# ZINZINBIN/Optimal-Control-1D-Electrostatic-Plasma

Hardware: AMD Instinct MI355X
Metric: particle-steps/sec (N×envs×steps) at N=1e6, Ng=256; % HBM roofline (higher is better)
Workload: dtype f64

## Files before the change

optimal-control-1d-electrostatic-plasma_amd/csrc/host_plan.h:

```cpp
#pragma once

#include <cmath>
#include <cstddef>
#include <cstdint>
#include <string>

#include "picstep.h"

#include "pic_limits.h"

enum Format : int { FMT_F64 = 0, FMT_F32 = 1, FMT_U32 = 2 };

struct LaunchPlan {
  int fmt = FMT_F64;
  int acc_kind = PIC_ACC_FIX64;
  int vec = 2;
  size_t esz = 8;
  long long ld = 0;
  long long chunk = 0;
  int nblk = 0;
  int R = 1;
  int fg = 42;
  int S = 1;
  double magic = 0;
  size_t sweep_lds = 0, solve_lds = 0;
  bool resident = false;
  int res_ppt = 0, res_nw = 0, res_R = 1;
  bool res_lean = false;
  size_t res_lds = 0;
  size_t res_carry_bytes = 0;
  double dx = 0, scale = 0;
  double cs[4]{}, ds[4]{};
  bool light_inner_steps = false;
  bool readonly_auto = false;
  size_t sweep_lds_rc = 0;
  bool v_separate = false;
  bool h_part_at_create = false;
  bool h_fields = false;
};

static inline void yoshida_coefficients(double (&c)[4], double (&d)[4]) {
  const double cbrt2 = std::pow(2.0, 1.0 / 3.0);
  const double w0 = (-1) * cbrt2 / (2 - cbrt2);
  const double w1 = 1 / (2 - cbrt2);
  c[0] = c[3] = 0.5 * w1;
  c[1] = c[2] = 0.5 * (w0 + w1);
  d[0] = 0.0;
  d[1] = d[3] = w1;
  d[2] = w0;
}

static inline int plan_fail(std::string* err, const std::string& msg) {
  if (err) *err = msg;
  return PIC_EINVAL;
}

static inline int check_config(const pic_config& c, std::string* err) {
  const pic_config* cfg = &c;
  if (cfg->N < 1 || cfg->Ng < 4 || cfg->num_envs < 1 || !(cfg->L > 0) || !(cfg->dt > 0) || !(cfg->n0 > 0))
    return plan_fail(err, "pic_create: need N>=1, Ng>=4, num_envs>=1, L>0, dt>0, n0>0");
  if (cfg->N > (1ll << 36)) return plan_fail(err, "pic_create: N > 2^36");
  if (cfg->num_envs > 65535) return plan_fail(err, "pic_create: num_envs > 65535");
  if (cfg->env_index_base < 0) return plan_fail(err, "pic_create: env_index_base < 0");
  if (cfg->particle_dtype != PIC_F64 && cfg->particle_dtype != PIC_F32)
    return plan_fail(err, "pic_create: particle_dtype must be PIC_F64 or PIC_F32");
  if (cfg->position_dtype != PIC_POS_FLOAT && cfg->position_dtype != PIC_POS_FIXED32)
    return plan_fail(err, "pic_create: position_dtype must be PIC_POS_FLOAT or PIC_POS_FIXED32");
  if (cfg->position_dtype == PIC_POS_FIXED32 && cfg->particle_dtype != PIC_F32)
    return plan_fail(err, "pic_create: 32-bit fixed-point positions go with float32 particles");
  if (cfg->accum_dtype < PIC_ACC_AUTO || cfg->accum_dtype > PIC_ACC_F64)
    return plan_fail(err, "pic_create: accum_dtype must be PIC_ACC_AUTO, _FIX64, _PACKED or _F64");
  if (cfg->interpol != PIC_CIC && cfg->interpol != PIC_TSC)
    return plan_fail(err, "pic_create: interpol must be PIC_CIC or PIC_TSC");
  if (cfg->accum_dtype == PIC_ACC_PACKED && cfg->particle_dtype != PIC_F32)
    return plan_fail(err, "pic_create: the packed accumulator needs float32 particles");
  if (cfg->accum_dtype == PIC_ACC_PACKED && cfg->interpol != PIC_CIC)
    return plan_fail(err, "pic_create: the packed accumulator is CIC only");
  if (cfg->placement != PIC_PLACE_AUTO && cfg->placement != PIC_PLACE_OFF)
    return plan_fail(err, "pic_create: placement must be PIC_PLACE_AUTO or PIC_PLACE_OFF");
  if (cfg->placement_ms < 0) return plan_fail(err, "pic_create: placement_ms < 0");
  if (cfg->accum_dtype == PIC_ACC_F64 && cfg->particle_dtype != PIC_F64)
    return plan_fail(err, "pic_create: the float64 accumulator needs float64 particles");
  return PIC_OK;
}

static inline int plan_launch(const pic_config& c, int ncu, LaunchPlan* p, std::string* err) {
  const pic_config* cfg = &c;
  *p = LaunchPlan{};
  p->fmt = cfg->particle_dtype == PIC_F64 ? FMT_F64 : (cfg->position_dtype == PIC_POS_FIXED32 ? FMT_U32 : FMT_F32);
  p->acc_kind = cfg->accum_dtype;
  if (p->acc_kind == PIC_ACC_AUTO)
    p->acc_kind = (cfg->particle_dtype == PIC_F32 && cfg->interpol == PIC_CIC) ? PIC_ACC_PACKED : PIC_ACC_FIX64;
  p->esz = cfg->particle_dtype == PIC_F64 ? 8 : 4;
  p->vec = cfg->particle_dtype == PIC_F64 ? 2 : 4;
  p->dx = cfg->L / cfg->Ng;
  p->scale = cfg->n0 * cfg->L / (double)cfg->N / p->dx;
  yoshida_coefficients(p->cs, p->ds);
  p->ld = (cfg->N + 63) / 64 * 64;
  int lg = 0;
  while ((1ll << lg) < cfg->N + 1) ++lg;
  p->fg = 62 - lg > 50 ? 50 : 62 - lg;
  p->magic = std::ldexp(1.5, 52 - p->fg);

  const long long tile = (long long)BLOCK * p->vec;
  long long nblk = cfg->blocks_per_env;
  if (nblk <= 0) {
    const long long target_total = 8192;
    nblk = (target_total + cfg->num_envs - 1) / cfg->num_envs;
    const bool small = (double)cfg->N * cfg->num_envs <= 4.0e6 && cfg->N <= 131072;
    long long tiles_min = small ? 1 : 8;
    if (!small && (cfg->N + 8 * tile - 1) / (8 * tile) * cfg->num_envs < 256) tiles_min = 4;
    long long max_by_work = (cfg->N + tiles_min * tile - 1) / (tiles_min * tile);
    if (small && max_by_work > 64) max_by_work = 64;
    if (nblk > max_by_work) nblk = max_by_work;
    if (nblk < 1) nblk = 1;
    const long long by10 = (cfg->N + 10 * tile - 1) / (10 * tile);
    if (!small && nblk < by10) nblk = by10;
    if (!small) {
      const long long by4 = (cfg->N + 4 * tile - 1) / (4 * tile);
      if (nblk * cfg->num_envs < 6ll * ncu) {
        for (long long k = 2; k <= 6; ++k) {
          long long c = k * ncu / cfg->num_envs;
          if (c > by4) c = by4;
          if (c >= nblk || c == by4) { nblk = c; break; }
        }
      }
    }
  }
  {
    const long long cap = (1ll << 27) - tile;
    if (nblk < (cfg->N + cap - 1) / cap) nblk = (cfg->N + cap - 1) / cap;
  }
  if (p->acc_kind == PIC_ACC_PACKED) {
    const long long cap = (1ll << 20) - tile;
    if (nblk < (cfg->N + cap - 1) / cap) nblk = (cfg->N + cap - 1) / cap;
  }
  long long chunk = (cfg->N + nblk - 1) / nblk;
  chunk = (chunk + tile - 1) / tile * tile;
  nblk = (cfg->N + chunk - 1) / chunk;
  if (nblk > 65535) return plan_fail(err, "pic_create: blocks_per_env too large");
  p->chunk = chunk;
  p->nblk = (int)nblk;
  p->light_inner_steps = 2.0 * (double)cfg->num_envs * (double)p->ld * (double)p->esz >= 256.0 * 1048576.0;
  p->readonly_auto = p->light_inner_steps;
  p->S = 1;
  while (p->S < 4 && nblk / (2 * p->S) >= 8 && (long long)cfg->num_envs * 2 * p->S <= 32) p->S *= 2;

  const size_t stride = (size_t)cfg->Ng + 2;
  p->R = 1;
  p->sweep_lds = 2 * p->R * stride * 8 + stride * p->esz;
  p->solve_lds = 2 * (size_t)cfg->Ng * sizeof(double);
  if (p->sweep_lds + stride * p->esz + kSweepStaticLds <= kLdsLimit) p->sweep_lds_rc = p->sweep_lds + stride * p->esz;
  else p->readonly_auto = false;
  if (p->sweep_lds + kSweepStaticLds > kLdsLimit) {
    const long long max_ng = (long long)((kLdsLimit - kSweepStaticLds) / (2 * p->R * 8 + p->esz)) - 2;
    return plan_fail(err, "pic_create: Ng too large for the LDS-resident mesh (at most " + std::to_string(max_ng) +
                                     " cells with this particle dtype)");
  }
  {
    static const int shapes[4][3] = {{8, 4, 2048}, {8, 8, 4096}, {8, 10, 5120}, {8, 16, 8192}};
    for (const auto& sh : shapes)
      if (cfg->N <= sh[2]) { p->res_nw = sh[0]; p->res_ppt = sh[1]; break; }
    p->res_R = 1;
    auto need = [&](int R) { return (size_t)2 * R * stride * 8 + 4 * (size_t)cfg->Ng * 8 + stride * p->esz; };
    while (p->res_R > 1 && need(p->res_R) > 48 * 1024) p->res_R >>= 1;
    p->res_lds = need(p->res_R);
    const bool possible = p->res_nw != 0 && p->res_lds + kResidentStaticLds <= kLdsLimit && p->acc_kind != PIC_ACC_F64;
    if (cfg->blocks_per_env < 0 && !possible) {
      const long long max_ng = (long long)((kLdsLimit - kResidentStaticLds - 2 * (2 * 8 + p->esz)) / (2 * 8 + p->esz + 4 * 8));
      return plan_fail(err, "pic_create: the resident schedule needs N <= 8192, Ng <= " + std::to_string(max_ng) +
                                       " (this particle dtype) and an integer accumulator");
    }
    const bool worth = cfg->N <= 5120 || cfg->num_envs >= 32;
    p->resident = possible && (cfg->blocks_per_env < 0 || (cfg->blocks_per_env == 0 && worth));
    p->res_lean = (cfg->num_envs > ncu && p->res_ppt <= 10) || (cfg->interpol == PIC_TSC && p->res_ppt == 16);
  }
  if (p->resident && !p->res_lean && p->res_ppt <= 10 && p->esz == 8 && cfg->num_envs <= 32)
    p->res_carry_bytes = (size_t)cfg->num_envs * p->res_nw * 64 * p->res_ppt * (sizeof(int) + (cfg->interpol == PIC_TSC ? 4 : 2) * p->esz);
  p->v_separate = 2 * ((size_t)cfg->num_envs * p->ld * p->esz) >= ((size_t)256 << 20) && cfg->placement != PIC_PLACE_OFF;
  p->h_part_at_create = 2 * (size_t)cfg->num_envs * cfg->N * p->esz <= ((size_t)4 << 20);
  p->h_fields = (size_t)cfg->num_envs * cfg->Ng * sizeof(double) <= ((size_t)256 << 10);
  return PIC_OK;
}
```

optimal-control-1d-electrostatic-plasma_amd/csrc/pic_device.h:

```cpp
#pragma once
#include <hip/hip_runtime.h>

#include <cmath>
#include <cstdint>
#include <type_traits>

#include "picstep.h"
#include "pic_limits.h"

namespace {

#ifndef PIC_STAMP
#define PIC_STAMP(slot) ((void)0)
#define PIC_STAMP_LOADS(slot) ((void)0)
#endif

constexpr int kInlineDoubles = 32;
struct InlineDoubles { double v[kInlineDoubles]; };

template <typename T>
__device__ __forceinline__ T kernarg_at(size_t offset) {
#if defined(__HIP_DEVICE_COMPILE__)
  using KP = const __attribute__((address_space(4))) char*;
  KP ka = (KP)__builtin_amdgcn_kernarg_segment_ptr();
  asm volatile("" : "+s"(ka));
  T out;
  __builtin_memcpy(&out, (const __attribute__((address_space(4))) T*)(ka + offset), sizeof(T));
  return out;
#else
  (void)offset;
  return T{};
#endif
}

template <typename T>
__device__ __forceinline__ const T* kernarg_ptr(size_t offset) {
#if defined(__HIP_DEVICE_COMPILE__)
  using KP = const __attribute__((address_space(4))) char*;
  KP ka = (KP)__builtin_amdgcn_kernarg_segment_ptr();
  return (const T*)(const char*)(ka + offset);
#else
  (void)offset;
  return nullptr;
#endif
}

template <int BYTES>
__device__ __forceinline__ void kernarg_warm() {
#if defined(__HIP_DEVICE_COMPILE__)
  using KP = const __attribute__((address_space(4))) unsigned*;
  KP ka = (KP)__builtin_amdgcn_kernarg_segment_ptr();
  unsigned w = 0;
#pragma unroll
  for (int line = 1; line < (BYTES + 63) / 64; ++line) w |= ka[line * 16];
  asm volatile("" ::"s"(w));
#endif
}

enum Stage : int {
  ST_A = 0,
  ST_B = 1,
  ST_C = 2,
  ST_D = 3,
  ST_REFRESH = 4,
  ST_PROBE = 5,
  ST_B2 = 6,
  ST_D2 = 7,
  ST_SE = 8,
  ST_FE = 9,
  ST_VK = 10,
  ST_VM = 11,
  ST_C_RO = 12,
  ST_D_RC = 13,
  ST_D2_RC = 14
};

using acc_t = long long;

__device__ __forceinline__ acc_t acc_row_sum(const acc_t* __restrict__ row, int j, int S, long long sub) {
  const acc_t* p = row + j;
  acc_t t = 0;
  int s = 0;
  for (; s + 4 <= S; s += 4) {
    const acc_t r0 = p[0]; p += sub;
    const acc_t r1 = p[0]; p += sub;
    const acc_t r2 = p[0]; p += sub;
    const acc_t r3 = p[0]; p += sub;
    t += (r0 + r1) + (r2 + r3);
  }
  for (; s < S; ++s) { t += p[0]; p += sub; }
  return t;
}

struct SweepArgs {
  long long N;
  long long ld;
  long long chunk;
  int Ng;
  int nblk;
  int R;
  int reverse;
  int fg;
  int S;
  int act_inline;
  long long sub;
  double magic;
  double L, dx, rdx, dt;
  double c_prev, c_cur, d_cur, c_next, d_prev;
  double scale, n0;
  double to_units;
  double N_over_L;
};

struct SolveArgs {
  long long N;
  long long sub;
  int Ng;
  int nblk;
  int fg;
  int S;
  double L, dx, n0;
  double scale;
  double N_over_L;
};

struct AccRequest { acc_t r[4]; };
__device__ __forceinline__ AccRequest acc_row_request(const acc_t* __restrict__ row, int j, int S, long long sub) {
  AccRequest q;
#pragma unroll
  for (int s = 0; s < 4; ++s) q.r[s] = row[(size_t)(s < S ? s : 0) * sub + j];
  return q;
}
__device__ __forceinline__ acc_t acc_row_finish(const AccRequest& q, int S) {
  return (q.r[0] + (S > 1 ? q.r[1] : 0)) + ((S > 2 ? q.r[2] : 0) + (S > 3 ? q.r[3] : 0));
}

struct Control {
  const double* ext;
  const double* act;
  const double* basis;
  int M;
};

__device__ __forceinline__ double actuator_field(const double* __restrict__ bc, const double* __restrict__ bs,
                                                 const double* __restrict__ a, int j, int M) {
  double c = 0.0, s = 0.0;
  for (int m = 0; m < M; ++m) c += bc[(size_t)j * M + m] * a[m];
  for (int m = 0; m < M; ++m) s += bs[(size_t)j * M + m] * a[M + m];
  return c + s;
}

typedef double pic_v2d __attribute__((ext_vector_type(2)));
typedef float pic_v4f __attribute__((ext_vector_type(4)));
typedef unsigned pic_v4u __attribute__((ext_vector_type(4)));

struct PosF64 { using X = double;   using V = double; using W = double; using XV = pic_v2d; using VV = pic_v2d; static constexpr int VEC = 2; static constexpr bool kFixed = false; };
struct PosF32 { using X = float;    using V = float;  using W = float;  using XV = pic_v4f; using VV = pic_v4f; static constexpr int VEC = 4; static constexpr bool kFixed = false; };
struct PosU32 { using X = unsigned; using V = float;  using W = float;  using XV = pic_v4u; using VV = pic_v4f; static constexpr int VEC = 4; static constexpr bool kFixed = true; };

template <typename VT>
__device__ __forceinline__ VT stream_load(const VT* p) { return *p; }

struct StreamOut {
  __amdgpu_buffer_rsrc_t rsrc;
  __device__ explicit StreamOut(void* base) : rsrc(__builtin_amdgcn_make_buffer_rsrc(base, 0, 0x7fffffff, 0x00020000)) {}
  template <typename VT>
  __device__ __forceinline__ void store(int off, VT v) const {
    static_assert(sizeof(VT) == 16, "particle tiles are 16 bytes per lane");
    typedef unsigned pic_v4raw __attribute__((ext_vector_type(4)));
    pic_v4raw w;
    __builtin_memcpy(&w, &v, 16);
    __builtin_amdgcn_raw_buffer_store_b128(w, rsrc, off, 0, 16);
  }
};

template <typename P>
struct Consts {
  typename P::W L, dx, rdx, dt, c_prev, c_cur, d_cur, c_next, d_prev;
  float to_units;
  double magic;
  int Ng;
  __device__ explicit Consts(const SweepArgs& a)
      : L((typename P::W)a.L), dx((typename P::W)a.dx), rdx((typename P::W)a.rdx), dt((typename P::W)a.dt),
        c_prev((typename P::W)a.c_prev), c_cur((typename P::W)a.c_cur), d_cur((typename P::W)a.d_cur),
        c_next((typename P::W)a.c_next), d_prev((typename P::W)a.d_prev), to_units((float)a.to_units), magic(a.magic), Ng(a.Ng) {}
  __device__ Consts(double L_, double dx_, int Ng_)
      : L((typename P::W)L_), dx((typename P::W)dx_), rdx((typename P::W)1 / (typename P::W)dx_), dt(0), c_prev(0),
        c_cur(0), d_cur(0), c_next(0), d_prev(0), to_units((float)(4294967296.0 / L_)), magic(0), Ng(Ng_) {}
};

template <typename T>
__device__ __noinline__ T wrap_periodic_far(T q, T L) {
  T r = fmod(q, L);
  if (r < T(0)) {
    r += L;
    if (r >= L) r = T(0);
  } else if (r == T(0)) {
    r = T(0);
  }
  return r;
}

template <typename T>
__device__ __forceinline__ T wrap_periodic(T q, T L, unsigned& bad) {
  if (__builtin_amdgcn_ballot_w64(!(q > T(0) && q < L)) == 0) return q;
  T up = q + L;
  up = (up >= L) ? T(0) : up;
  T r = (q <= T(0)) ? up : q;
  r = (q >= L) ? q - L : r;
  if (__builtin_expect(!(r >= T(0) && r < L), 0)) {
    r = wrap_periodic_far(q, L);
    if (!(r >= T(0) && r < L)) {
      bad += 1u;
      r = T(0);
    }
  }
  return r;
}

template <typename T>
__device__ __forceinline__ T div_dx(T a, T dx, T rdx) {
  T q0 = a * rdx;
  T rem = fma(-q0, dx, a);
  return fma(rem, rdx, q0);
}

template <typename P, int SHAPE>
__device__ __forceinline__ void locate_in_box(typename P::X xw, const Consts<P>& k, int& j, typename P::W (&w)[3], unsigned& frac) {
  using T = typename P::W;
  static_assert(!P::kFixed, "fixed-point positions need no wrap: locate() is the whole of it");
  frac = 0u;
  T jf = floor(div_dx(xw, k.dx, k.rdx));
  j = (int)jf;
  if ((unsigned)j >= (unsigned)k.Ng) j = 0;
  if (SHAPE == PIC_CIC) {
    w[0] = div_dx((jf + T(1)) * k.dx - xw, k.dx, k.rdx);
    w[1] = div_dx(xw - jf * k.dx, k.dx, k.rdx);
    w[2] = T(0);
  } else {
    T d = div_dx(xw - jf * k.dx, k.dx, k.rdx);
    T a = T(1.5) - d, b = d - T(1), c = d - T(0.5);
    w[0] = T(0.5) * (a * a);
    w[1] = T(0.75) - b * b;
    w[2] = T(0.5) * (c * c);
  }
}

template <typename P, int SHAPE>
__device__ __forceinline__ void locate(typename P::X q, const Consts<P>& k, typename P::X& xw, int& j,
                                       typename P::W (&w)[3], unsigned& frac, unsigned& bad) {
  using T = typename P::W;
  if constexpr (P::kFixed) {
    xw = q;
    j = (int)__umulhi(q, (unsigned)k.Ng);
    frac = q * (unsigned)k.Ng;
    const T d = (T)frac * T(2.3283064365386963e-10);
    if (SHAPE == PIC_CIC) {
      w[1] = d;
      w[0] = T(1) - d;
      w[2] = T(0);
    } else {
      T a = T(1.5) - d, b = d - T(1), c = d - T(0.5);
      w[0] = T(0.5) * (a * a);
      w[1] = T(0.75) - b * b;
      w[2] = T(0.5) * (c * c);
    }
  } else {
    xw = wrap_periodic(q, k.L, bad);
    locate_in_box<P, SHAPE>(xw, k, j, w, frac);
  }
}

template <typename P>
__device__ __forceinline__ double pos_to_length(typename P::X q, double L) {
  if constexpr (P::kFixed) return (double)q * (L * 2.3283064365386963e-10);
  else return (double)q;
}

template <typename P>
__device__ __forceinline__ typename P::X pos_from_length(double xs, double L, unsigned& bad) {
  if constexpr (P::kFixed) {
    double r = xs - floor(xs / L) * L;
    if (!(r >= 0.0 && r < L)) { if (!(r == L)) bad += 1u; r = 0.0; }
    return (unsigned)((unsigned long long)rint(r / L * 4294967296.0) & 0xFFFFFFFFull);
  } else {
    return (typename P::X)xs;
  }
}

template <typename P>
__device__ __forceinline__ typename P::X drift(typename P::X q, typename P::V p, typename P::W c, const Consts<P>& k,
                                               unsigned& bad) {
  using T = typename P::W;
  if constexpr (P::kFixed) {
    const float d = ((c * (T)p) * k.dt) * k.to_units;
    if (!(fabsf(d) < 2147483648.0f)) bad += 1u;
    return q + (unsigned)__float2int_rn(d);
  } else {
    return q + (c * (T)p) * k.dt;
  }
}

template <typename T, int SHAPE>
__device__ __forceinline__ T gather_field(const T* __restrict__ Es, int j, const T (&w)[3]) {
  T e = w[0] * Es[j] + w[1] * Es[j + 1];
  if (SHAPE == PIC_TSC) e = e + w[2] * Es[j + 2];
  return e;
}

struct fix_t { unsigned long long v; };
constexpr int FX_FRAC = 24;
constexpr int FX_LOW = 44;

__device__ __forceinline__ acc_t to_fixed(double w, double magic) {
  return __double_as_longlong(w + magic) - __double_as_longlong(magic);
}

template <typename A, typename P, int SHAPE>
__device__ __forceinline__ void deposit(A* __restrict__ acc, int j, const typename P::W (&w)[3], unsigned frac,
                                        double magic) {
  if constexpr (std::is_same<A, fix_t>::value) {
    static_assert(SHAPE == PIC_CIC, "the packed accumulator is CIC only");
    unsigned long long lo;
    if constexpr (P::kFixed) {
      lo = (frac >> 8) + ((frac >> 7) & 1u);
    } else {
      const float wr = fminf(fmaxf((float)w[1], 0.0f), 1.0f);
      lo = (unsigned long long)(unsigned)(wr * (float)(1u << FX_FRAC) + 0.5f);
    }
    atomicAdd(reinterpret_cast<unsigned long long*>(acc) + j, (1ull << FX_LOW) + lo);
  } else if constexpr (std::is_same<A, acc_t>::value) {
    unsigned long long* a = reinterpret_cast<unsigned long long*>(acc);
    atomicAdd(a + j, (unsigned long long)to_fixed((double)w[0], magic));
    atomicAdd(a + j + 1, (unsigned long long)to_fixed((double)w[1], magic));
    if (SHAPE == PIC_TSC) atomicAdd(a + j + 2, (unsigned long long)to_fixed((double)w[2], magic));
  } else {
    atomicAdd(&acc[j], (A)w[0]);
    atomicAdd(&acc[j + 1], (A)w[1]);
    if (SHAPE == PIC_TSC) atomicAdd(&acc[j + 2], (A)w[2]);
  }
}

template <int CTRL, int ROW_MASK = 0xF>
__device__ __forceinline__ double dpp_add(double v) {
  const int lo = __builtin_amdgcn_update_dpp(0, __double2loint(v), CTRL, ROW_MASK, 0xF, true);
  const int hi = __builtin_amdgcn_update_dpp(0, __double2hiint(v), CTRL, ROW_MASK, 0xF, true);
  return v + __hiloint2double(hi, lo);
}

__device__ __forceinline__ double wave_incl_scan(double v) {
  v = dpp_add<0x111>(v);
  v = dpp_add<0x112>(v);
  v = dpp_add<0x114>(v);
  v = dpp_add<0x118>(v);
  v = dpp_add<0x142, 0xA>(v);
  v = dpp_add<0x143, 0xC>(v);
  return v;
}

__device__ __forceinline__ double wave_sum(double v) {
  v = wave_incl_scan(v);
  const int lo = __builtin_amdgcn_readlane(__double2loint(v), 63);
  const int hi = __builtin_amdgcn_readlane(__double2hiint(v), 63);
  return __hiloint2double(hi, lo);
}

template <int NW>
__device__ __forceinline__ double block_excl_scan(double v, double* ws, double& total) {
  const int lane = threadIdx.x & 63, w = threadIdx.x >> 6;
  double inc = wave_incl_scan(v);
  if (lane == 63) ws[w] = inc;
  __syncthreads();
  double off = 0.0, tot = 0.0;
  for (int i = 0; i < NW; ++i) {
    double s = ws[i];
    if (i < w) off += s;
    tot += s;
  }
  __syncthreads();
  total = tot;
  return off + (inc - v);
}

template <int NW>
__device__ __forceinline__ double block_sum(double v, double* ws) {
  double w = wave_sum(v);
  if ((threadIdx.x & 63) == 0) ws[threadIdx.x >> 6] = w;
  __syncthreads();
  double s = 0.0;
  for (int i = 0; i < NW; ++i) s += ws[i];
  __syncthreads();
  return s;
}

template <int NW>
__device__ __forceinline__ void block_sum2(double a, double b, double* ws, double& sa, double& sb) {
  const double wa = wave_sum(a), wb = wave_sum(b);
  if ((threadIdx.x & 63) == 0) {
    ws[threadIdx.x >> 6] = wa;
    ws[NW + (threadIdx.x >> 6)] = wb;
  }
  __syncthreads();
  sa = 0.0;
  sb = 0.0;
  for (int i = 0; i < NW; ++i) {
    sa += ws[i];
    sb += ws[NW + i];
  }
  __syncthreads();
}

template <int NW>
__device__ __forceinline__ void mesh_mode(const double* __restrict__ E, const double* __restrict__ twc,
                                          const double* __restrict__ tws, int Ng, double* __restrict__ ws, double& re,
                                          double& im) {
  double sr = 0.0, si = 0.0;
  int t0 = threadIdx.x;
  asm volatile("" : "+v"(t0));
  for (int j = t0; j < Ng; j += NW * 64) {
    const double e = E[j];
    sr += e * twc[j];
    si -= e * tws[j];
  }
  double a, b;
  block_sum2<NW>(sr, si, ws, a, b);
  re = a / Ng * 2.0;
  im = b / Ng * 2.0;
}

struct Feedback {
  const double* tw;
  int rows;
  int M;
  double* act_out;
  double* act_hist;
  const double* gain;
  double* modes;
  double* modes_hist;
};

__device__ __forceinline__ double gain_row(const double* __restrict__ g, const double* __restrict__ m, int n) {
  double acc = 0.0;
  bool any = false;
  for (int k = 0; k < n; ++k) {
    const double gk = g[k];
    if (gk != 0.0) {
      const double t = gk * m[k];
      acc = any ? acc + t : t;
      any = true;
    }
  }
  return acc;
}

template <int NW>
__device__ __forceinline__ void feedback_action(const double* __restrict__ E, const Feedback& fb, int env, int Ng,
                                                double* __restrict__ ws, double* __restrict__ a_lds) {
  const size_t r = (size_t)env * 2 * fb.M;
  for (int m = 0; m < fb.M; ++m) {
    double re, im;
    mesh_mode<NW>(E, fb.tw + (size_t)m * Ng, fb.tw + ((size_t)fb.rows + m) * Ng, Ng, ws, re, im);
    if (threadIdx.x == 0) {
      if (fb.gain) {
        double* mv = a_lds ? a_lds : fb.modes + r;
        mv[m] = re; mv[fb.M + m] = im;
        if (fb.modes_hist) { fb.modes_hist[r + m] = re; fb.modes_hist[r + fb.M + m] = im; }
        continue;
      }
      const double c = -re, s = im;
      if (a_lds) { a_lds[m] = c; a_lds[fb.M + m] = s; }
      if (fb.act_out) { fb.act_out[r + m] = c; fb.act_out[r + fb.M + m] = s; }
      if (fb.act_hist) { fb.act_hist[r + m] = c; fb.act_hist[r + fb.M + m] = s; }
    }
  }
  if (fb.gain) {
    __syncthreads();
    const int n = 2 * fb.M;
    int i = threadIdx.x;
    asm volatile("" : "+v"(i));
    const double a = i < n ? gain_row(fb.gain + (r + i) * n, a_lds ? a_lds : fb.modes + r, n) : 0.0;
    if (a_lds) __syncthreads();
    if (i < n) {
      if (a_lds) a_lds[i] = a;
      if (fb.act_out) fb.act_out[r + i] = a;
      if (fb.act_hist) fb.act_hist[r + i] = a;
    }
  }
}

__device__ __forceinline__ void scan_fields(double* __restrict__ sb, double* __restrict__ sp, int Ng, double dx,
                                            double* __restrict__ slot, int wave = 0) {
  if ((int)(threadIdx.x >> 6) != wave) return;
  const int lane = threadIdx.x & 63;
  const int m = (Ng + 63) / 64;
  const int lo = min(lane * m, Ng), hi = min(lo + m, Ng);
  double loc = 0.0;
  for (int j = lo; j < hi; ++j) loc += sb[j];
  double run = wave_incl_scan(loc) - loc;
  loc = 0.0;
  for (int j = lo; j < hi; ++j) {
    run += sb[j];
    const double g = run * dx;
    sb[j] = g;
    loc += g;
  }
  const double gmean = wave_sum(loc) / (double)Ng;
  if (lane == 0) slot[0] = gmean;
  if (sp) {
    loc = 0.0;
    for (int j = lo; j < hi; ++j) loc += (sb[j] - gmean) * dx;
    run = wave_incl_scan(loc) - loc;
    double ploc = 0.0;
    for (int j = lo; j < hi; ++j) {
      sp[j] = run;
      ploc += run;
      run += (sb[j] - gmean) * dx;
    }
    ploc = wave_sum(ploc);
    if (lane == 0) slot[1] = ploc / (double)Ng;
  }
}

struct SolveOut {
  const double* ext;
  double *E, *phi;
  double *KE, *PE, *PEr;
  double* hist;
  int num_envs;
  Feedback fb;
};

template <int NW>
__device__ __forceinline__ void solve_block(const SolveOut& o, int env, int Ng, double dx, double N_over_L, double ke_share,
                                            double* __restrict__ sb, double* __restrict__ se, double* __restrict__ ws,
                                            double* __restrict__ slot) {
  constexpr int NT = NW * 64;
  const int tid = threadIdx.x;
  const size_t row = (size_t)env * Ng;
  scan_fields(sb, o.phi ? se : nullptr, Ng, dx, slot);
  __syncthreads();
  const double gmean = slot[0];
  const double pmean = o.phi ? slot[1] : 0.0;
  double e2 = 0.0;
  for (int j = tid; j < Ng; j += NT) {
    const double gp = sb[j] - gmean;
    const double gm = sb[j == 0 ? Ng - 1 : j - 1] - gmean;
    const double E = -0.5 * (gp + gm);
    const double Et = o.ext ? E + o.ext[row + j] : E;
    if (o.E) o.E[row + j] = Et;
    e2 += Et * Et;
    if (o.phi) o.phi[row + j] = se[j] - pmean;
  }
  double S, K;
  block_sum2<NW>(e2, ke_share, ws, S, K);
  if (tid == 0) {
    const double pe = 0.5 * S * dx;
    if (o.PEr) o.PEr[env] = pe;
    if (o.PE) o.PE[env] = pe * N_over_L;
    if (o.KE) o.KE[env] = 0.5 * K;
    if (o.hist) {
      o.hist[env] = 0.5 * K;
      o.hist[o.num_envs + env] = pe * N_over_L;
      o.hist[2 * (size_t)o.num_envs + env] = pe;
    }
  }
  if (o.fb.M > 0) feedback_action<NW>(o.E + row, o.fb, env, Ng, ws, nullptr);
}

}
```

optimal-control-1d-electrostatic-plasma_amd/csrc/pic_sweep.h:

```cpp
#pragma once
#include "pic_device.h"
#include "pic_solve.h"

namespace {

template <typename T, int OFF>
__device__ __forceinline__ void prologue_field(const acc_t* __restrict__ acc_in, const AccRequest& first, int S, long long sub,
                                               const Control& ctl, double* __restrict__ ext_out, int Ng, double unit, double scale,
                                               double n0, double dx, double* __restrict__ sb, double* __restrict__ xt,
                                               double* __restrict__ slot, T* __restrict__ Es) {
  const int tid = threadIdx.x;
  if (ctl.act)
    for (int j = tid; j < Ng; j += BLOCK) {
      const double e = actuator_field(ctl.basis, ctl.basis + (size_t)Ng * ctl.M, ctl.act, j, ctl.M);
      xt[j] = e;
      if (ext_out) ext_out[j] = e;
    }
  if (tid < Ng) sb[tid] = ((double)acc_row_finish(first, S) * unit) * scale - n0;
  for (int j = tid + BLOCK; j < Ng; j += BLOCK)
    sb[j] = ((double)acc_row_sum(acc_in, j, S, sub) * unit) * scale - n0;
  __syncthreads();
  PIC_STAMP(3);
  scan_fields(sb, nullptr, Ng, dx, slot);
  __syncthreads();
  PIC_STAMP(4);
  const double gmean = slot[0];
  for (int i = tid; i < Ng + 2; i += BLOCK) {
    int node = i - OFF;
    node = node < 0 ? node + Ng : (node >= Ng ? node - Ng : node);
    const double gp = sb[node] - gmean;
    const double gm = sb[node == 0 ? Ng - 1 : node - 1] - gmean;
    double E = -0.5 * (gp + gm);
    if (ctl.act) E += xt[node];
    else if (ctl.ext) E += ctl.ext[node];
    Es[i] = (T)E;
  }
  __syncthreads();
  PIC_STAMP(5);
}

template <typename P, int SHAPE>
__device__ __forceinline__ void substage(typename P::X& q, typename P::V& p, const typename P::W* __restrict__ Es,
                                         typename P::W d, typename P::W c, const Consts<P>& k, unsigned& bad) {
  using T = typename P::W;
  T w[3];
  typename P::X xw;
  int j;
  unsigned frac;
  locate<P, SHAPE>(q, k, xw, j, w, frac, bad);
  const T E = gather_field<T, SHAPE>(Es, j, w);
  p = p + (typename P::V)((d * (-E)) * k.dt);
  q = drift<P>(q, p, c, k, bad);
}

template <typename P, typename A, int SHAPE, int STAGE>
__device__ __forceinline__ void push_one(typename P::X& xq, typename P::V& vp, const typename P::W* __restrict__ Es,
                                         const typename P::W* __restrict__ Es2, A* __restrict__ acc, A* __restrict__ acc2,
                                         const Consts<P>& k, double& ke, unsigned& bad) {
  constexpr bool kC = (STAGE == ST_C || STAGE == ST_C_RO);
  constexpr bool kRC = (STAGE == ST_D_RC || STAGE == ST_D2_RC);
  constexpr bool kD = (STAGE == ST_D || STAGE == ST_D_RC);
  constexpr bool kD2 = (STAGE == ST_D2 || STAGE == ST_D2_RC);
  using T = typename P::W;
  T w[3];
  typename P::X xw;
  int j;
  unsigned frac;
  typename P::X q = xq;
  typename P::V p = vp;
  if (kRC) {
    unsigned again = 0u;
    substage<P, SHAPE>(q, p, Es2, k.d_prev, k.c_prev, k, again);
  }
  if (STAGE == ST_B2) {
    if constexpr (P::kFixed) locate<P, SHAPE>(q, k, xw, j, w, frac, bad);
    else locate_in_box<P, SHAPE>(q, k, j, w, frac);
    deposit<A, P, SHAPE>(acc2, j, w, frac, k.magic);
  }
  if (STAGE == ST_A) {
    q = drift<P>(q, p, k.c_cur, k, bad);
  } else if (STAGE == ST_B || STAGE == ST_B2 || kC || kD || kD2) {
    if (STAGE == ST_B || STAGE == ST_B2) q = drift<P>(q, p, k.c_prev, k, bad);
    substage<P, SHAPE>(q, p, Es, k.d_cur, k.c_cur, k, bad);
  }
  if (kD2) {
    if constexpr (P::kFixed) xw = q;
    else xw = wrap_periodic(q, k.L, bad);
  } else {
    locate<P, SHAPE>(q, k, xw, j, w, frac, bad);
    deposit<A, P, SHAPE>(acc, j, w, frac, k.magic);
  }
  if (kD || kD2 || STAGE == ST_REFRESH) {
    q = xw;
    ke += (double)p * (double)p;
    const typename P::X qn = drift<P>(q, p, k.c_next, k, bad);
    typename P::X xn;
    locate<P, SHAPE>(qn, k, xn, j, w, frac, bad);
    deposit<A, P, SHAPE>(acc2, j, w, frac, k.magic);
  }
  xq = q;
  vp = p;
}

template <typename P, typename A, int SHAPE, int STAGE>
__device__ __forceinline__ void push_scheme(typename P::X& xq, typename P::V& vp, const typename P::W* __restrict__ Es,
                                            A* __restrict__ acc, const Consts<P>& k, double& ke, unsigned& bad) {
  using T = typename P::W;
  using V = typename P::V;
  T w[3];
  typename P::X xw;
  int j;
  unsigned frac;
  typename P::X q = xq;
  V p = vp;
  locate<P, SHAPE>(q, k, xw, j, w, frac, bad);
  const T E = gather_field<T, SHAPE>(Es, j, w);
  if (STAGE == ST_FE) {
    q = drift<P>(xw, p, k.c_cur, k, bad);
    p = p + (V)((k.d_cur * (-E)) * k.dt);
  } else {
    p = p + (V)((k.d_cur * (-E)) * k.dt);
    if (STAGE == ST_VK || STAGE == ST_VM) {
      q = xw;
      ke += (double)p * (double)p;
    }
    if (STAGE == ST_VM) p = p + (V)((k.d_cur * (-E)) * k.dt);
    if (STAGE != ST_VK) q = drift<P>(q, p, k.c_cur, k, bad);
  }
  if (STAGE != ST_VK) {
    locate<P, SHAPE>(q, k, xw, j, w, frac, bad);
    deposit<A, P, SHAPE>(acc, j, w, frac, k.magic);
    if (STAGE != ST_VM) {
      q = xw;
      ke += (double)p * (double)p;
    }
  }
  xq = q;
  vp = p;
}

template <typename A, int SHAPE>
__device__ __forceinline__ acc_t mesh_node_sum(const A* __restrict__ acc_all, int R, int stride, int Ng, int fg, int c) {
  constexpr int OFF = (SHAPE == PIC_TSC) ? 1 : 0;
  if constexpr (std::is_same<A, fix_t>::value) {
    const unsigned long long* a = reinterpret_cast<const unsigned long long*>(acc_all);
    const int cm = c == 0 ? Ng - 1 : c - 1;
    unsigned long long own = 0ull, left = 0ull;
    for (int r = 0; r < R; ++r) {
      own += a[(size_t)r * stride + c];
      left += a[(size_t)r * stride + cm];
    }
    const long long mask = (1ll << FX_LOW) - 1;
    const long long q = ((long long)(own >> FX_LOW) << FX_FRAC) - ((long long)own & mask) + ((long long)left & mask);
    return q << (fg - FX_FRAC);
  } else {
    A s = A(0);
    for (int r = 0; r < R; ++r) {
      const A* ar = acc_all + (size_t)r * stride;
      A t = ar[c + OFF];
      if (SHAPE == PIC_CIC) {
        if (c == 0) t += ar[Ng];
      } else {
        if (c == 0) t += ar[Ng + 1];
        if (c == Ng - 1) t += ar[0];
      }
      s += t;
    }
    if constexpr (std::is_same<A, acc_t>::value) return s;
    else return __double2ll_rn(ldexp((double)s, fg));
  }
}

template <typename A, int SHAPE>
__device__ __forceinline__ void flush_mesh(const A* __restrict__ acc_all, int R, int stride, int Ng, int fg,
                                           acc_t* __restrict__ row) {
  unsigned long long* out = reinterpret_cast<unsigned long long*>(row);
  for (int c = threadIdx.x; c < Ng; c += BLOCK) {
    const acc_t q = mesh_node_sum<A, SHAPE>(acc_all, R, stride, Ng, fg, c);
    if (q) atomicAdd(out + c, (unsigned long long)q);
  }
}

struct SweepIO {
  const acc_t* acc_in;
  Control ctl;
  double* ext_out;
  const double* next_act;
  acc_t* acc_out;
  acc_t* acc_out2;
  acc_t* zero0;
  acc_t* zero1;
  double* ke_part;
  unsigned long long* bad;
  SolveIO post;
  double* e2;
};

constexpr size_t kSweepInlineOffset = 2 * sizeof(void*) + sizeof(SweepIO) + sizeof(SweepArgs);
static_assert(sizeof(SweepIO) % 8 == 0 && sizeof(SweepArgs) % 8 == 0, "arguments lie back to back");

template <typename P, typename A, int SHAPE, int STAGE>
__global__ __launch_bounds__(BLOCK) void sweep_kernel(typename P::X* __restrict__ x, typename P::V* __restrict__ v,
                                                      SweepIO io, SweepArgs a, InlineDoubles act_inline) {
  constexpr int OFF = (SHAPE == PIC_TSC) ? 1 : 0;
  constexpr int VEC = P::VEC;
  using T = typename P::W;
  using XV = typename P::XV;
  using VV = typename P::VV;
  constexpr bool kIsB = (STAGE == ST_B || STAGE == ST_B2), kIsC = (STAGE == ST_C || STAGE == ST_C_RO);
  constexpr bool kRC = (STAGE == ST_D_RC || STAGE == ST_D2_RC);
  constexpr bool kIsD = (STAGE == ST_D || STAGE == ST_D2 || kRC);
  constexpr bool kScheme = (STAGE >= ST_SE && STAGE <= ST_VM);
  constexpr bool kGather = (kIsB || kIsC || kIsD || kScheme);
  constexpr bool kStore = ((kGather && STAGE != ST_C_RO) || STAGE == ST_REFRESH);
  constexpr bool kStoreV = kGather && STAGE != ST_C_RO;
  constexpr bool kAhead = !kStore;
  constexpr bool kReadV = (STAGE != ST_PROBE);
  constexpr bool kFirst = (STAGE != ST_D2 && STAGE != ST_D2_RC && STAGE != ST_VK);
  constexpr bool kDual = (kIsD || STAGE == ST_REFRESH || STAGE == ST_B2);
  constexpr bool kEnergy = (kIsD || STAGE == ST_REFRESH || kScheme);

  extern __shared__ __align__(16) unsigned char smem_raw[];
  const int Ng = a.Ng;
  const int stride = Ng + 2;
  A* acc_all = reinterpret_cast<A*>(smem_raw);
  A* acc2_all = acc_all + (size_t)a.R * stride;
  T* Es = reinterpret_cast<T*>(smem_raw + (size_t)2 * a.R * stride * sizeof(A));
  T* Es2 = Es + stride;
  __shared__ double red[2 * WAVES];
  __shared__ double slot[2];
  static_assert(sizeof(red) + sizeof(slot) == kSweepStaticLds, "pic_create adds the static LDS to the dynamic part it sizes");
  PIC_STAMP(0);

  if (kIsC && blockIdx.x == (unsigned)a.nblk) {
    SolveIO post = kernarg_at<SolveIO>(2 * sizeof(void*) + offsetof(SweepIO, post));
    post.out.fb = Feedback{};
    solve_environment(post, blockIdx.y, Ng, a.nblk, a.fg, a.S, a.sub, a.scale, a.n0, a.dx, a.N_over_L, smem_raw, red, slot);
    return;
  }

  const int tid = threadIdx.x;
  const int env = a.reverse ? (int)gridDim.y - 1 - (int)blockIdx.y : (int)blockIdx.y;
  const int blk = a.reverse ? a.nblk - 1 - (int)blockIdx.x : (int)blockIdx.x;

  typename P::X* xe = x + (size_t)env * a.ld;
  typename P::V* ve = v + (size_t)env * a.ld;
  const long long step = (long long)BLOCK * VEC;
  const long long begin = (long long)blk * a.chunk;
  long long end = begin + a.chunk;
  if (end > a.N) end = a.N;
  long long i = begin + (long long)tid * VEC;
  AccRequest first_node{};
  if (kGather) first_node = acc_row_request(io.acc_in + (size_t)env * Ng, tid < Ng ? tid : Ng - 1, a.S, a.sub);
  const long long i_first = (i + VEC <= end) ? i : 0;
  XV xv = stream_load(reinterpret_cast<const XV*>(xe + i_first));
  VV vv = {};
  if (kReadV) vv = stream_load(reinterpret_cast<const VV*>(ve + i_first));
  PIC_STAMP(2);

  bool clear_first = true;
  if (kGather) {
    Control ctl = io.ctl;
    if (ctl.ext) ctl.ext += (size_t)env * Ng;
    if (a.act_inline) ctl.act = kernarg_ptr<double>(kSweepInlineOffset);
    if (ctl.act) ctl.act += (size_t)env * 2 * ctl.M;
    else {
      for (int c = tid; c < a.R * stride; c += BLOCK) acc_all[c] = A{};
      clear_first = false;
    }
    prologue_field<T, OFF>(io.acc_in + (size_t)env * Ng, first_node, a.S, a.sub, ctl,
                           (io.ext_out && blk == 0) ? io.ext_out + (size_t)env * Ng : nullptr, Ng, ldexp(1.0, -a.fg), a.scale, a.n0, a.dx,
                           reinterpret_cast<double*>(acc2_all), reinterpret_cast<double*>(smem_raw), slot, Es);
  }
  if (STAGE == ST_C_RO && blk == 0)
    for (int c = tid; c < stride; c += BLOCK) io.e2[(size_t)env * stride + c] = (double)Es[c];
  if (kRC)
    for (int c = tid; c < stride; c += BLOCK) Es2[c] = (T)io.e2[(size_t)env * stride + c];
  if (kIsD && io.next_act && io.ext_out && blk == 0) {
    const Control ctl = io.ctl;
    for (int j = tid; j < Ng; j += BLOCK)
      io.ext_out[(size_t)env * Ng + j] = actuator_field(ctl.basis, ctl.basis + (size_t)Ng * ctl.M, io.next_act + (size_t)env * 2 * ctl.M, j, ctl.M);
  }
  if (clear_first) for (int c = tid; c < a.R * stride; c += BLOCK) acc_all[c] = A{};
  if (kDual) for (int c = tid; c < a.R * stride; c += BLOCK) acc2_all[c] = A{};
  if (blk < a.S) {
    const size_t z = (size_t)blk * a.sub + (size_t)env * Ng;
    if (io.zero0) for (int c = tid; c < Ng; c += BLOCK) io.zero0[z + c] = 0;
    if (io.zero1) for (int c = tid; c < Ng; c += BLOCK) io.zero1[z + c] = 0;
  }
  if (clear_first || kDual) __syncthreads();
  PIC_STAMP(6);

  const int rep = (tid >> 6) & (a.R - 1);
  A* acc = acc_all + (size_t)rep * stride;
  A* acc2 = acc2_all + (size_t)rep * stride;
  const Consts<P> k(a);

  double ke = 0.0;
  unsigned bad = 0u;
  [[maybe_unused]] int tile = 0;
  const StreamOut xout(xe + begin), vout(ve + begin);
  while (i + VEC <= end) {
    PIC_STAMP_LOADS(8 + 2 * tile);
    [[maybe_unused]] XV xv_next;
    [[maybe_unused]] VV vv_next = {};
    if constexpr (kAhead) {
      const long long i_next = (i + step + VEC <= end) ? i + step : 0;
      xv_next = stream_load(reinterpret_cast<const XV*>(xe + i_next));
      if (kReadV) vv_next = stream_load(reinterpret_cast<const VV*>(ve + i_next));
    }
    typename P::X* xs = reinterpret_cast<typename P::X*>(&xv);
    typename P::V* vs = reinterpret_cast<typename P::V*>(&vv);
#pragma unroll
    for (int c = 0; c < VEC; ++c) {
      typename P::V pv = kReadV ? vs[c] : typename P::V(0);
      if constexpr (kScheme) push_scheme<P, A, SHAPE, STAGE>(xs[c], pv, Es, acc, k, ke, bad);
      else push_one<P, A, SHAPE, STAGE>(xs[c], pv, Es, Es2, acc, acc2, k, ke, bad);
      if (kReadV) vs[c] = pv;
    }
    if (kStore) {
      xout.store((int)((i - begin) * (long long)sizeof(typename P::X)), xv);
      if (kStoreV) vout.store((int)((i - begin) * (long long)sizeof(typename P::V)), vv);
    }
    PIC_STAMP(9 + 2 * tile);
    ++tile;
    i += step;
    if constexpr (kAhead) {
      xv = xv_next;
      vv = vv_next;
    } else if (i + VEC <= end) {
      xv = stream_load(reinterpret_cast<const XV*>(xe + i));
      if (kReadV) vv = stream_load(reinterpret_cast<const VV*>(ve + i));
    }
  }
  for (long long c = i; c < end; ++c) {
    typename P::X xq = xe[c];
    typename P::V pv = kReadV ? ve[c] : typename P::V(0);
    if constexpr (kScheme) push_scheme<P, A, SHAPE, STAGE>(xq, pv, Es, acc, k, ke, bad);
    else push_one<P, A, SHAPE, STAGE>(xq, pv, Es, Es2, acc, acc2, k, ke, bad);
    if (kStore) {
      xe[c] = xq;
      if (kStoreV) ve[c] = pv;
    }
  }
  __syncthreads();
  PIC_STAMP(24);

  const size_t sub_row = (size_t)(blk % a.S) * a.sub + (size_t)env * Ng;
  if (kFirst) flush_mesh<A, SHAPE>(acc_all, a.R, stride, Ng, a.fg, io.acc_out + sub_row);
  if (kDual) flush_mesh<A, SHAPE>(acc2_all, a.R, stride, Ng, a.fg, io.acc_out2 + sub_row);
  PIC_STAMP(25);

  if (kEnergy) {
    double w = wave_sum(ke);
    if ((tid & 63) == 0) red[tid >> 6] = w;
    __syncthreads();
    if (tid == 0) {
      double s = 0.0;
      for (int c = 0; c < WAVES; ++c) s += red[c];
      io.ke_part[(size_t)env * a.nblk + blk] = s;
    }
  }
  if (bad) atomicAdd(io.bad, (unsigned long long)bad);
  PIC_STAMP_LOADS(26);
}

}
```

Measured before the change: 76.71 billion.

## Trim particle push inner loop: unfolded CIC index, cheaper fixed-point convert, double-buffered tile loads

Adds a ping-pong double-buffered main loop that loads the next particle tile through scalar base plus vector lane offset addressing while pushing the current one, replacing the per-tile prefetch loop for most tiles. For CIC with non-fixed accumulators it skips folding the out-of-range cell index, and instead has the mesh flush pick up the extra ghost node. It also makes to_fixed subtract only the high 32-bit word of the magic constant, with a host check that the low word is zero. The periodic wrap is restructured to a single return path. A profiling summary script is included as well.

Measured after the change: 77.64 billion (median of 6 runs). +1.2%, better.

```diff
diff --git a/optimal-control-1d-electrostatic-plasma_amd/csrc/host_plan.h b/optimal-control-1d-electrostatic-plasma_amd/csrc/host_plan.h
--- a/optimal-control-1d-electrostatic-plasma_amd/csrc/host_plan.h
+++ b/optimal-control-1d-electrostatic-plasma_amd/csrc/host_plan.h
@@ -3,6 +3,7 @@
 #include <cmath>
 #include <cstddef>
 #include <cstdint>
+#include <cstring>
 #include <string>
 
 #include "picstep.h"
@@ -101,6 +102,11 @@
   while ((1ll << lg) < cfg->N + 1) ++lg;
   p->fg = 62 - lg > 50 ? 50 : 62 - lg;
   p->magic = std::ldexp(1.5, 52 - p->fg);
+  {
+    std::uint64_t bits;
+    std::memcpy(&bits, &p->magic, sizeof(bits));
+    if ((bits & 0xffffffffull) != 0) return plan_fail(err, "pic_create: the fixed-point magic has a non-zero low word");
+  }
 
   const long long tile = (long long)BLOCK * p->vec;
   long long nblk = cfg->blocks_per_env;
diff --git a/optimal-control-1d-electrostatic-plasma_amd/csrc/pic_device.h b/optimal-control-1d-electrostatic-plasma_amd/csrc/pic_device.h
--- a/optimal-control-1d-electrostatic-plasma_amd/csrc/pic_device.h
+++ b/optimal-control-1d-electrostatic-plasma_amd/csrc/pic_device.h
@@ -203,16 +203,18 @@
 
 template <typename T>
 __device__ __forceinline__ T wrap_periodic(T q, T L, unsigned& bad) {
-  if (__builtin_amdgcn_ballot_w64(!(q > T(0) && q < L)) == 0) return q;
-  T up = q + L;
-  up = (up >= L) ? T(0) : up;
-  T r = (q <= T(0)) ? up : q;
-  r = (q >= L) ? q - L : r;
-  if (__builtin_expect(!(r >= T(0) && r < L), 0)) {
-    r = wrap_periodic_far(q, L);
-    if (!(r >= T(0) && r < L)) {
-      bad += 1u;
-      r = T(0);
+  T r = q;
+  if (__builtin_amdgcn_ballot_w64(!(q > T(0) && q < L)) != 0) {
+    T up = q + L;
+    up = (up >= L) ? T(0) : up;
+    r = (q <= T(0)) ? up : q;
+    r = (q >= L) ? q - L : r;
+    if (__builtin_expect(!(r >= T(0) && r < L), 0)) {
+      r = wrap_periodic_far(q, L);
+      if (!(r >= T(0) && r < L)) {
+        bad += 1u;
+        r = T(0);
+      }
     }
   }
   return r;
@@ -225,14 +227,14 @@
   return fma(rem, rdx, q0);
 }
 
-template <typename P, int SHAPE>
+template <typename P, int SHAPE, bool FOLD = true>
 __device__ __forceinline__ void locate_in_box(typename P::X xw, const Consts<P>& k, int& j, typename P::W (&w)[3], unsigned& frac) {
   using T = typename P::W;
   static_assert(!P::kFixed, "fixed-point positions need no wrap: locate() is the whole of it");
   frac = 0u;
   T jf = floor(div_dx(xw, k.dx, k.rdx));
   j = (int)jf;
-  if ((unsigned)j >= (unsigned)k.Ng) j = 0;
+  if (FOLD && (unsigned)j >= (unsigned)k.Ng) j = 0;
   if (SHAPE == PIC_CIC) {
     w[0] = div_dx((jf + T(1)) * k.dx - xw, k.dx, k.rdx);
     w[1] = div_dx(xw - jf * k.dx, k.dx, k.rdx);
@@ -246,7 +248,7 @@
   }
 }
 
-template <typename P, int SHAPE>
+template <typename P, int SHAPE, bool FOLD = true>
 __device__ __forceinline__ void locate(typename P::X q, const Consts<P>& k, typename P::X& xw, int& j,
                                        typename P::W (&w)[3], unsigned& frac, unsigned& bad) {
   using T = typename P::W;
@@ -267,7 +269,7 @@
     }
   } else {
     xw = wrap_periodic(q, k.L, bad);
-    locate_in_box<P, SHAPE>(xw, k, j, w, frac);
+    locate_in_box<P, SHAPE, FOLD>(xw, k, j, w, frac);
   }
 }
 
@@ -312,8 +314,12 @@
 constexpr int FX_FRAC = 24;
 constexpr int FX_LOW = 44;
 
+typedef int pic_v2i __attribute__((ext_vector_type(2)));
+
 __device__ __forceinline__ acc_t to_fixed(double w, double magic) {
-  return __double_as_longlong(w + magic) - __double_as_longlong(magic);
+  pic_v2i s = __builtin_bit_cast(pic_v2i, w + magic);
+  s.y -= __builtin_bit_cast(pic_v2i, magic).y;
+  return __builtin_bit_cast(acc_t, s);
 }
 
 template <typename A, typename P, int SHAPE>
diff --git a/optimal-control-1d-electrostatic-plasma_amd/csrc/pic_sweep.h b/optimal-control-1d-electrostatic-plasma_amd/csrc/pic_sweep.h
--- a/optimal-control-1d-electrostatic-plasma_amd/csrc/pic_sweep.h
+++ b/optimal-control-1d-electrostatic-plasma_amd/csrc/pic_sweep.h
@@ -39,7 +39,10 @@
   PIC_STAMP(5);
 }
 
-template <typename P, int SHAPE>
+template <typename A, int SHAPE>
+constexpr bool kFoldIndex = !(SHAPE == PIC_CIC && !std::is_same<A, fix_t>::value);
+
+template <typename P, int SHAPE, bool FOLD>
 __device__ __forceinline__ void substage(typename P::X& q, typename P::V& p, const typename P::W* __restrict__ Es,
                                          typename P::W d, typename P::W c, const Consts<P>& k, unsigned& bad) {
   using T = typename P::W;
@@ -47,7 +50,7 @@
   typename P::X xw;
   int j;
   unsigned frac;
-  locate<P, SHAPE>(q, k, xw, j, w, frac, bad);
+  locate<P, SHAPE, FOLD>(q, k, xw, j, w, frac, bad);
   const T E = gather_field<T, SHAPE>(Es, j, w);
   p = p + (typename P::V)((d * (-E)) * k.dt);
   q = drift<P>(q, p, c, k, bad);
@@ -61,6 +64,7 @@
   constexpr bool kRC = (STAGE == ST_D_RC || STAGE == ST_D2_RC);
   constexpr bool kD = (STAGE == ST_D || STAGE == ST_D_RC);
   constexpr bool kD2 = (STAGE == ST_D2 || STAGE == ST_D2_RC);
+  constexpr bool kFold = kFoldIndex<A, SHAPE>;
   using T = typename P::W;
   T w[3];
   typename P::X xw;
@@ -70,7 +74,7 @@
   typename P::V p = vp;
   if (kRC) {
     unsigned again = 0u;
-    substage<P, SHAPE>(q, p, Es2, k.d_prev, k.c_prev, k, again);
+    substage<P, SHAPE, kFold>(q, p, Es2, k.d_prev, k.c_prev, k, again);
   }
   if (STAGE == ST_B2) {
     if constexpr (P::kFixed) locate<P, SHAPE>(q, k, xw, j, w, frac, bad);
@@ -81,13 +85,13 @@
     q = drift<P>(q, p, k.c_cur, k, bad);
   } else if (STAGE == ST_B || STAGE == ST_B2 || kC || kD || kD2) {
     if (STAGE == ST_B || STAGE == ST_B2) q = drift<P>(q, p, k.c_prev, k, bad);
-    substage<P, SHAPE>(q, p, Es, k.d_cur, k.c_cur, k, bad);
+    substage<P, SHAPE, kFold>(q, p, Es, k.d_cur, k.c_cur, k, bad);
   }
   if (kD2) {
     if constexpr (P::kFixed) xw = q;
     else xw = wrap_periodic(q, k.L, bad);
   } else {
-    locate<P, SHAPE>(q, k, xw, j, w, frac, bad);
+    locate<P, SHAPE, kFold>(q, k, xw, j, w, frac, bad);
     deposit<A, P, SHAPE>(acc, j, w, frac, k.magic);
   }
   if (kD || kD2 || STAGE == ST_REFRESH) {
@@ -95,7 +99,7 @@
     ke += (double)p * (double)p;
     const typename P::X qn = drift<P>(q, p, k.c_next, k, bad);
     typename P::X xn;
-    locate<P, SHAPE>(qn, k, xn, j, w, frac, bad);
+    locate<P, SHAPE, kFold>(qn, k, xn, j, w, frac, bad);
     deposit<A, P, SHAPE>(acc2, j, w, frac, k.magic);
   }
   xq = q;
@@ -113,7 +117,8 @@
   unsigned frac;
   typename P::X q = xq;
   V p = vp;
-  locate<P, SHAPE>(q, k, xw, j, w, frac, bad);
+  constexpr bool kFold = kFoldIndex<A, SHAPE>;
+  locate<P, SHAPE, kFold>(q, k, xw, j, w, frac, bad);
   const T E = gather_field<T, SHAPE>(Es, j, w);
   if (STAGE == ST_FE) {
     q = drift<P>(xw, p, k.c_cur, k, bad);
@@ -128,7 +133,7 @@
     if (STAGE != ST_VK) q = drift<P>(q, p, k.c_cur, k, bad);
   }
   if (STAGE != ST_VK) {
-    locate<P, SHAPE>(q, k, xw, j, w, frac, bad);
+    locate<P, SHAPE, kFold>(q, k, xw, j, w, frac, bad);
     deposit<A, P, SHAPE>(acc, j, w, frac, k.magic);
     if (STAGE != ST_VM) {
       q = xw;
@@ -139,7 +144,7 @@
   vp = p;
 }
 
-template <typename A, int SHAPE>
+template <typename A, int SHAPE, bool WIDE = false>
 __device__ __forceinline__ acc_t mesh_node_sum(const A* __restrict__ acc_all, int R, int stride, int Ng, int fg, int c) {
   constexpr int OFF = (SHAPE == PIC_TSC) ? 1 : 0;
   if constexpr (std::is_same<A, fix_t>::value) {
@@ -160,6 +165,7 @@
       A t = ar[c + OFF];
       if (SHAPE == PIC_CIC) {
         if (c == 0) t += ar[Ng];
+        if (WIDE && c == 1) t += ar[Ng + 1];
       } else {
         if (c == 0) t += ar[Ng + 1];
         if (c == Ng - 1) t += ar[0];
@@ -176,7 +182,7 @@
                                            acc_t* __restrict__ row) {
   unsigned long long* out = reinterpret_cast<unsigned long long*>(row);
   for (int c = threadIdx.x; c < Ng; c += BLOCK) {
-    const acc_t q = mesh_node_sum<A, SHAPE>(acc_all, R, stride, Ng, fg, c);
+    const acc_t q = mesh_node_sum<A, SHAPE, !kFoldIndex<A, SHAPE>>(acc_all, R, stride, Ng, fg, c);
     if (q) atomicAdd(out + c, (unsigned long long)q);
   }
 }
@@ -300,6 +306,65 @@
   unsigned bad = 0u;
   [[maybe_unused]] int tile = 0;
   const StreamOut xout(xe + begin), vout(ve + begin);
+  if constexpr (kAhead) {
+    const int nfull = (int)((end - begin) / step);
+    if (nfull >= 2) {
+      using GlobalBytes = const __attribute__((address_space(1))) char*;
+      GlobalBytes xp = (GlobalBytes) reinterpret_cast<const char*>(xe + begin);
+      GlobalBytes vp = (GlobalBytes) reinterpret_cast<const char*>(ve + begin);
+      unsigned lane_off = (unsigned)tid * (unsigned)sizeof(XV);
+      asm("" : "+v"(lane_off));
+      constexpr size_t kTileBytes = (size_t)BLOCK * sizeof(XV);
+      static_assert(sizeof(XV) == sizeof(VV), "one lane offset serves both streams");
+      auto tile_x = [&](GlobalBytes base) __attribute__((always_inline)) {
+        asm("" : "+s"(base));
+        return *reinterpret_cast<const __attribute__((address_space(1))) XV*>(base + lane_off);
+      };
+      auto tile_v = [&](GlobalBytes base) __attribute__((always_inline)) {
+        asm("" : "+s"(base));
+        return *reinterpret_cast<const __attribute__((address_space(1))) VV*>(base + lane_off);
+      };
+      auto push_tile = [&](XV& xt, VV& vt) __attribute__((always_inline)) {
+        typename P::X* xs = reinterpret_cast<typename P::X*>(&xt);
+        typename P::V* vs = reinterpret_cast<typename P::V*>(&vt);
+#pragma unroll
+        for (int c = 0; c < VEC; ++c) {
+          typename P::V pv = kReadV ? vs[c] : typename P::V(0);
+          push_one<P, A, SHAPE, STAGE>(xs[c], pv, Es, Es2, acc, acc2, k, ke, bad);
+        }
+      };
+      XV xw;
+      VV vw = {};
+      int left = nfull - 1;
+      for (; left >= 2; left -= 2) {
+        PIC_STAMP_LOADS(8 + 2 * tile);
+        xw = tile_x(xp + kTileBytes);
+        if (kReadV) vw = tile_v(vp + kTileBytes);
+        push_tile(xv, vv);
+        PIC_STAMP(9 + 2 * tile);
+        ++tile;
+        xp += 2 * kTileBytes;
+        vp += 2 * kTileBytes;
+        PIC_STAMP_LOADS(8 + 2 * tile);
+        xv = tile_x(xp);
+        if (kReadV) vv = tile_v(vp);
+        push_tile(xw, vw);
+        PIC_STAMP(9 + 2 * tile);
+        ++tile;
+      }
+      if (left) {
+        PIC_STAMP_LOADS(8 + 2 * tile);
+        xw = tile_x(xp + kTileBytes);
+        if (kReadV) vw = tile_v(vp + kTileBytes);
+        push_tile(xv, vv);
+        PIC_STAMP(9 + 2 * tile);
+        ++tile;
+        xv = xw;
+        vv = vw;
+      }
+      i += (long long)(nfull - 1) * step;
+    }
+  }
   while (i + VEC <= end) {
     PIC_STAMP_LOADS(8 + 2 * tile);
     [[maybe_unused]] XV xv_next;
diff --git a/profiles/pmc_sum.py b/profiles/pmc_sum.py
--- /dev/null
+++ b/profiles/pmc_sum.py
@@ -0,0 +1,15 @@
+import collections, csv, glob, os, re, sys
+d, tag = sys.argv[1:3]
+agg = collections.defaultdict(list)
+for f in glob.glob(os.path.join(d, "**", "*_counter_collection.csv"), recursive=True):
+    for r in csv.DictReader(open(f)):
+        m = re.search(r"sweep_kernel<.*?,\s*(\d+)>", r["Kernel_Name"])
+        if m:
+            agg[(r["Counter_Name"], int(m.group(1)))].append(float(r["Counter_Value"]))
+for (c, s), v in sorted(agg.items()):
+    print(tag, c, "stage", s, "launches", len(v), "mean", sum(v) / len(v))
+for f in glob.glob(os.path.join(d, "**", "*_kernel_stats.csv"), recursive=True):
+    for r in csv.DictReader(open(f)):
+        m = re.search(r"sweep_kernel<.*?,\s*(\d+)>", r["Name"])
+        if m:
+            print(tag, "kernel_stats stage", m.group(1), "calls", r["Calls"], "avg_ns", r["AverageNs"], "min_ns", r["MinNs"], "max_ns", r["MaxNs"])
```
